# shihchinw/rlShaders

Hardware: AMD Instinct MI355X
Metric: BSDF Gsamples/sec (eval+sample+pdf) (higher is better)
Workload: dtype f32

## Files before the change

### rlshaders_amd/build.py

```python
from __future__ import annotations

import os
import shutil
import subprocess
import sys
from concurrent.futures import ThreadPoolExecutor
from pathlib import Path

PKG = Path(__file__).resolve().parent
CSRC = PKG / "csrc"
LIBDIR = PKG / "lib"
OBJDIR = PKG / "build"
LIB = LIBDIR / "librlshaders_amd.so"
ARCH = "gfx950"

SOURCES = ["shade.hip", "integrate.hip", "lights.hip", "scatter.hip", "skin.hip", "ggx.hip", "disney.hip", "sss.hip", "alternates.hip", "context.hip", "pipeline.hip",
           "libm_check.hip"]
FAST_UNITS = {"ggx.hip", "disney.hip", "sss.hip", "skin.hip", "integrate.hip", "lights.hip", "scatter.hip", "shade.hip", "alternates.hip"}
HEADERS = [CSRC / "rls_device.hpp", CSRC / "rls_libm.hpp", CSRC / "rls_libm_tables.inc", CSRC / "rls_libm_flavour_args.inc", CSRC / "rls_internal.hpp", CSRC / "rls_loops.hpp",
           PKG.parent / "include" / "rlshaders_amd.h", PKG.parent / "include" / "rlshaders_amd_diag.h"]

HIPCC_FLAGS = [
    f"--offload-arch={ARCH}", "-O3", "-std=c++17", "-fPIC",
    "-ffp-contract=off", "-fno-fast-math",
    "-fno-slp-vectorize",
    "-fno-gpu-rdc",
    "-Wall", "-Wno-unused-function",
]


def _hipcc() -> str:
    exe = shutil.which("hipcc") or "/opt/rocm/bin/hipcc"
    if not os.path.exists(exe):
        raise RuntimeError("hipcc not found: the rlshaders_amd HIP library cannot be built")
    return exe


def _stale(target: Path, deps) -> bool:
    if not target.exists():
        return True
    t = target.stat().st_mtime
    return any(Path(d).stat().st_mtime > t for d in deps)


def sources():
    return [CSRC / s for s in SOURCES if (CSRC / s).exists()]


def build_library(force: bool = False, verbose: bool = False, variant: str = "", defines=(), extra=()) -> Path:
    hipcc = _hipcc()
    LIBDIR.mkdir(exist_ok=True)
    objdir = OBJDIR if not variant else PKG / f"build_{variant}"
    lib = LIB if not variant else LIBDIR / f"librlshaders_amd_{variant}.so"
    objdir.mkdir(exist_ok=True)
    srcs = sources()
    jobs = []
    objs = []
    for src in srcs:
        flavours = [("", "RLS_FAST=0")] + ([("_fast", "RLS_FAST=1")] if src.name in FAST_UNITS else [])
        for suffix, flag in flavours:
            obj = objdir / (src.stem + suffix + ".o")
            objs.append(obj)
            if force or _stale(obj, [src, *HEADERS, Path(__file__)]):
                jobs.append([hipcc, *HIPCC_FLAGS, *extra, f"-cuid=rlshaders_amd.{src.stem}{suffix}", f"-D{flag}",
                             *[f"-D{d}" for d in defines], "-c", str(src), "-o", str(obj)])

    def run(cmd):
        if verbose:
            print(" ".join(cmd), flush=True)
        p = subprocess.run(cmd, capture_output=True, text=True)
        if p.returncode != 0:
            raise RuntimeError(f"hipcc failed:\n{' '.join(cmd)}\n{p.stdout}\n{p.stderr}")
        return p

    if jobs:
        with ThreadPoolExecutor(max_workers=min(4, len(jobs))) as ex:
            list(ex.map(run, jobs))
    if force or jobs or _stale(lib, objs):
        run([hipcc, f"--offload-arch={ARCH}", "-shared", "-fPIC", "-o", str(lib), *map(str, objs)])
    return lib


TRACE_CSRC = PKG / "csrc_trace"
TRACE_SOURCES = ["trace.hip"]
TRACE_LIB = LIBDIR / "librls_trace.so"
TRACE_HEADERS = [TRACE_CSRC / "rls_trace_device.hpp", PKG.parent / "include" / "rlshaders_amd_trace.h"]


def build_trace_library(force: bool = False, verbose: bool = False) -> Path:
    hipcc = _hipcc()
    main = build_library(verbose=verbose)
    objdir = OBJDIR / "trace"
    objdir.mkdir(parents=True, exist_ok=True)
    jobs, objs = [], []
    for name in TRACE_SOURCES:
        src = TRACE_CSRC / name
        for suffix, flag in (("", "RLS_FAST=0"), ("_fast", "RLS_FAST=1")):
            obj = objdir / (src.stem + suffix + ".o")
            objs.append(obj)
            if force or _stale(obj, [src, *HEADERS, *TRACE_HEADERS, Path(__file__)]):
                jobs.append([hipcc, *HIPCC_FLAGS, f"-cuid=rls_trace.{src.stem}{suffix}", f"-D{flag}", "-c", str(src),
                             "-o", str(obj)])

    def run(cmd):
        if verbose:
            print(" ".join(cmd), flush=True)
        p = subprocess.run(cmd, capture_output=True, text=True)
        if p.returncode != 0:
            raise RuntimeError(f"hipcc failed:\n{' '.join(cmd)}\n{p.stdout}\n{p.stderr}")

    if jobs:
        with ThreadPoolExecutor(max_workers=min(4, len(jobs))) as ex:
            list(ex.map(run, jobs))
    if force or jobs or _stale(TRACE_LIB, [*objs, main]):
        run([hipcc, f"--offload-arch={ARCH}", "-shared", "-fPIC", "-o", str(TRACE_LIB), *map(str, objs),
             f"-L{LIBDIR}", "-lrlshaders_amd", "-Wl,-rpath,$ORIGIN"])
    return TRACE_LIB


def build_trace_example(verbose: bool = False) -> Path:
    OBJDIR.mkdir(exist_ok=True)
    lib = build_trace_library(verbose=verbose)
    src, out = PKG / "host" / "example_trace.cpp", OBJDIR / "example_trace"
    if _stale(out, [src, PKG / "host" / "rls_trace.hpp", lib, LIB, *HEADERS, *TRACE_HEADERS]):
        cmd = ["g++", "-std=c++14", "-O2", "-Wall", f"-I{PKG.parent / 'include'}", f"-I{PKG / 'host'}", str(src), "-o", str(out),
               f"-L{LIBDIR}", "-lrls_trace", "-lrlshaders_amd", f"-Wl,-rpath,{LIBDIR}", "-L/opt/rocm/lib", "-Wl,-rpath,/opt/rocm/lib"]
        if verbose:
            print(" ".join(cmd), flush=True)
        p = subprocess.run(cmd, capture_output=True, text=True)
        if p.returncode != 0:
            raise RuntimeError(f"host example example_trace failed to build:\n{p.stdout}\n{p.stderr}")
    return out


def build_host_examples(verbose: bool = False) -> Path:
    OBJDIR.mkdir(exist_ok=True)
    first = OBJDIR / "example_arnold_stub"
    for name in ("example_arnold_stub", "example_multi_gpu", "example_host_pipeline", "test_arnold_stub"):
        src = PKG / "host" / f"{name}.cpp"
        out = OBJDIR / name
        if not src.exists():
            continue
        if _stale(out, [src, PKG / "host" / "rls_batch.hpp", PKG / "host" / "rl_arnold_stub.hpp", LIB, *HEADERS]):
            cmd = ["g++", "-std=c++14", "-O2", "-Wall", "-pthread", f"-I{PKG.parent / 'include'}", f"-I{PKG / 'host'}",
                   str(src), "-o", str(out), f"-L{LIBDIR}", "-lrlshaders_amd", f"-Wl,-rpath,{LIBDIR}",
                   "-L/opt/rocm/lib", "-Wl,-rpath,/opt/rocm/lib"]
            if verbose:
                print(" ".join(cmd), flush=True)
            p = subprocess.run(cmd, capture_output=True, text=True)
            if p.returncode != 0:
                raise RuntimeError(f"host example {name} failed to build:\n{p.stdout}\n{p.stderr}")
    return first


if __name__ == "__main__":
    args = sys.argv[1:]
    variant = args[args.index("--variant") + 1] if "--variant" in args else ""
    defines = [a[2:] for a in args if a.startswith("-D")]
    extra = []
    for i, a in enumerate(args):
        if a.startswith(("-f", "-m", "-O")):
            extra.append(a)
            if a == "-mllvm":
# ... 3 lines not shown
```

### rlshaders_amd/csrc/context.hip

```cpp
#include <stdarg.h>
#include <stdlib.h>
#include <string.h>

#include "rls_internal.hpp"

namespace {
thread_local char g_error[512] = "";
}

namespace rlsh {

void set_error(const char *fmt, ...)
{
    va_list ap;
    va_start(ap, fmt);
    vsnprintf(g_error, sizeof(g_error), fmt, ap);
    va_end(ap);
}

rls_status hip_fail(hipError_t e, const char *what)
{
    set_error("HIP error %d (%s) in %s", (int)e, hipGetErrorString(e), what);
    (void)hipGetLastError();
    return e == hipErrorOutOfMemory ? RLS_ERR_OUT_OF_MEMORY : RLS_ERR_HIP;
}

}

using namespace rlsd;

extern "C" {

const char *rls_last_error(void) { return g_error; }

const char *rls_status_string(rls_status s)
{
    switch (s) {
    case RLS_OK: return "ok";
    case RLS_ERR_INVALID_ARGUMENT: return "invalid argument";
    case RLS_ERR_NO_DEVICE: return "no HIP device";
    case RLS_ERR_HIP: return "HIP runtime error";
    case RLS_ERR_OUT_OF_MEMORY: return "out of device memory";
    case RLS_ERR_UNSUPPORTED: return "unsupported";
    case RLS_ERR_ABORTED: return "stopped by a callback";
    default: return "unknown status";
    }
}

int rls_version(void) { return RLS_VERSION_MAJOR * 1000 + RLS_VERSION_MINOR; }

rls_status rls_context_create(int device_ordinal, rls_context **out)
{
    RLS_REQUIRE(out != nullptr, "out is NULL");
    *out = nullptr;
    int count = 0;
    hipError_t e = hipGetDeviceCount(&count);
    if (e != hipSuccess || count <= 0) {
        rlsh::set_error("rls_context_create: no HIP device visible (%s)",
                        e == hipSuccess ? "count = 0" : hipGetErrorString(e));
        return RLS_ERR_NO_DEVICE;
    }
    if (device_ordinal < 0 || device_ordinal >= count) {
        rlsh::set_error("rls_context_create: device %d out of range [0, %d)", device_ordinal, count);
        return RLS_ERR_NO_DEVICE;
    }
    RLS_HIP_TRY(hipSetDevice(device_ordinal));
    hipDeviceProp_t prop;
    RLS_HIP_TRY(hipGetDeviceProperties(&prop, device_ordinal));

    rls_context *ctx = (rls_context *)calloc(1, sizeof(rls_context));
    if (!ctx) { rlsh::set_error("rls_context_create: host allocation failed"); return RLS_ERR_OUT_OF_MEMORY; }
    ctx->device = device_ordinal;
    ctx->compute_units = prop.multiProcessorCount > 0 ? prop.multiProcessorCount : 256;
    ctx->blocks_per_cu = 64;
    if (const char *s = getenv("RLS_BLOCKS_PER_CU")) {
        int v = atoi(s);
        if (v >= 1 && v <= 4096) ctx->blocks_per_cu = v;
    }
    hipError_t e1 = hipStreamCreateWithFlags(&ctx->own_stream, hipStreamNonBlocking);
    hipError_t e2 = e1 == hipSuccess ? hipEventCreate(&ctx->ev_start) : e1;
    hipError_t e3 = e2 == hipSuccess ? hipEventCreate(&ctx->ev_stop) : e2;
    if (e3 == hipSuccess) e3 = hipEventCreate(&ctx->ev_probe_start);
    if (e3 == hipSuccess) e3 = hipEventCreate(&ctx->ev_probe_stop);
    hipError_t e4 = e3 == hipSuccess ? hipMalloc((void **)&ctx->scratch_u64, sizeof(unsigned long long)) : e3;
    if (e4 != hipSuccess) {
        rls_status st = rlsh::hip_fail(e4, "rls_context_create");
        rls_context_destroy(ctx);
        return st;
    }
    ctx->stream = ctx->own_stream;
    *out = ctx;
    return RLS_OK;
}

void rls_context_destroy(rls_context *ctx)
{
    if (!ctx) return;
    (void)hipSetDevice(ctx->device);
    if (ctx->capturing) {
        hipGraph_t g = nullptr;
        if (hipStreamEndCapture(ctx->stream, &g) == hipSuccess && g) (void)hipGraphDestroy(g);
        (void)hipGetLastError();
    }
    if (ctx->own_stream) (void)hipStreamSynchronize(ctx->own_stream);
    if (ctx->scratch_u64) (void)hipFree(ctx->scratch_u64);
    if (ctx->stamp_buf) (void)hipFree(ctx->stamp_buf);
    if (ctx->ev_start) (void)hipEventDestroy(ctx->ev_start);
    if (ctx->ev_stop) (void)hipEventDestroy(ctx->ev_stop);
    if (ctx->ev_probe_start) (void)hipEventDestroy(ctx->ev_probe_start);
    if (ctx->ev_probe_stop) (void)hipEventDestroy(ctx->ev_probe_stop);
    if (ctx->own_stream) (void)hipStreamDestroy(ctx->own_stream);
    free(ctx);
}

int rls_device_count(void)
{
    int n = 0;
    if (hipGetDeviceCount(&n) != hipSuccess) { (void)hipGetLastError(); return 0; }
    return n;
}

rls_status rls_shard_range(int64_t total, int rank, int world, int64_t *first, int64_t *count)
{
    RLS_REQUIRE(first != nullptr && count != nullptr, "NULL argument");
    RLS_REQUIRE(world >= 1 && rank >= 0 && rank < world && total >= 0, "bad shard request");
    const __int128 lo = (__int128)total * rank / world, hi = (__int128)total * (rank + 1) / world;
    *first = (int64_t)lo;
    *count = (int64_t)(hi - lo);
    return RLS_OK;
}

rls_status rls_context_set_stream(rls_context *ctx, void *hip_stream)
{
    RLS_REQUIRE(ctx != nullptr, "ctx is NULL");
    RLS_REQUIRE(!ctx->capturing, "not allowed while a launch graph is being recorded");
    ctx->stream = (hipStream_t)hip_stream;
    return RLS_OK;
}

rls_status rls_context_use_own_stream(rls_context *ctx)
{
    RLS_REQUIRE(ctx != nullptr, "ctx is NULL");
    RLS_REQUIRE(!ctx->capturing, "not allowed while a launch graph is being recorded");
    ctx->stream = ctx->own_stream;
    return RLS_OK;
}

void *rls_context_get_stream(rls_context *ctx) { return ctx ? (void *)ctx->stream : nullptr; }

rls_status rls_context_set_math_mode(rls_context *ctx, int mode)
{
    RLS_REQUIRE(ctx != nullptr, "ctx is NULL");
    RLS_REQUIRE(mode == RLS_MATH_EXACT || mode == RLS_MATH_FAST, "mode must be RLS_MATH_EXACT or RLS_MATH_FAST");
    ctx->fast = mode == RLS_MATH_FAST;
    return RLS_OK;
}

int rls_context_get_math_mode(const rls_context *ctx) { return ctx && ctx->fast ? RLS_MATH_FAST : RLS_MATH_EXACT; }

int rls_context_device(const rls_context *ctx) { return ctx ? ctx->device : -1; }

// ... 496 lines not shown
```

### rlshaders_amd/csrc/ggx.hip

```cpp
#include "rls_internal.hpp"

using namespace rlsd;

namespace {

using namespace rlsh;

#define RLS_GGX_ARGS(a0) reload_args(a0)

enum { MIXED = 0, STREAMED_ALL = 1, UNIFORM_MATERIAL = 2 };

template <int MODE>
__device__ __forceinline__ Ggx load_closure(const rls_ggx_closure &c, Idx i, const GgxMaterial &um)
{
    constexpr bool STREAMED = MODE == STREAMED_ALL;
    V3 wo = ld3(c.wo, i), N = ld3(c.N, i), T = ld3(c.T, i);
    const PIndex<Idx> k = pindex<MODE == MIXED>(c.materials, i);
    float kr, kg, kb;
    ldrgb<STREAMED>(c.KsColor, k, kr, kg, kb);
    if (MODE == UNIFORM_MATERIAL)
        return ggx_from_material(um, wo, N, T, c.exiting ? (c.exiting[i.full()] != 0) : false, kr, kg, kb);
    float rough = ldp<STREAMED>(c.specularRoughness, k);
    float ior = ldp<STREAMED>(c.ior, k);
    float aniso = ldp<STREAMED>(c.anisotropic, k);
    bool exiting = c.exiting ? (c.exiting[i.full()] != 0) : false;
    return ggx_make(wo, N, T, exiting, kr, kg, kb, ior, rough, aniso);
}

#ifndef RLS_GGX_WAVES
#define RLS_GGX_WAVES(OP) ((OP) == OP_EVAL ? 6 : 8)
#endif
#define RLS_GGX_ATTR(OP) __launch_bounds__(rlsh::kBlock) __attribute__((amdgpu_waves_per_eu(RLS_GGX_WAVES(OP), RLS_GGX_WAVES(OP))))
template <int OP, int FAST_MATH, int MODE>
__device__ __forceinline__ void ggx_body(const GgxIO &a0)
{
    if (OP == OP_SAMPLE || OP == OP_FUSED || OP == OP_REFLECT_REFRACT || OP == OP_REFRACT || OP == OP_MICROFACET)
        stage_libm_tables();
    GgxMaterial um = {};
    if (MODE == UNIFORM_MATERIAL) {
        const rls_ggx_closure &c = a0.c;
        um = ggx_material_wave_uniform(ggx_material(c.ior.u, c.specularRoughness.u, c.anisotropic.u));
    }
    const TileRange tiles = tile_range(a0.n);
    for (int64_t base = tiles.first; base < tiles.end; base += tiles.step) {
        const Idx i = make_idx(base);
        if (i.full() >= a0.n) continue;
        const GgxIO a = RLS_GGX_ARGS(a0);
        Ggx g = load_closure<MODE>(a.c, i, um);

        if (OP == OP_SAMPLE || OP == OP_FUSED || OP == OP_REFLECT_REFRACT) {
            float rx = ldg(a.rx, i), ry = ldg(a.ry, i);
            VndfView w = vndf_view(g.view, g.fr, g.ax, g.ay);
            V3 M, M2;
            if (OP == OP_REFLECT_REFRACT) {
                float rx2 = ldg(a.rx2, i), ry2 = ldg(a.ry2, i);
                vndf_microfacet_pair(w, g.fr, rx, ry, w, g.fr, rx2, ry2, M, M2);
            } else {
                M = vndf_microfacet(w, g.fr, rx, ry);
            }
            V3 L = reflect_direction(g.view, M);
            float F = ggx_fresnel(g, L, M);
            {
                const GgxIO b = RLS_GGX_ARGS(a0);
                st3(b.wi, i, L);
                if (b.fresnel) stg(b.fresnel, i, F);
            }
            if (OP != OP_SAMPLE) {
                float fr, fg, fb, pdf;
                ggx_eval_pdf<true, true>(g, L, fr, fg, fb, pdf);
                const GgxIO b = RLS_GGX_ARGS(a0);
                strgb(b.f, i, fr, fg, fb);
                stg(b.pdf, i, pdf);
            }
            if (OP == OP_REFLECT_REFRACT) {
                V3 dir;
                ggx_refract(g, M2, dir);
                const float wgt = ggx_sample_weight(g, g.view, dir, M2);
                const GgxIO b = RLS_GGX_ARGS(a0);
                st3(b.wt, i, dir);
                stg(b.weight, i, wgt);
            }
        } else if (OP == OP_EVAL) {
            float fr, fg, fb;
            ggx_eval(g, ld3(a.cwi, i), fr, fg, fb);
            strgb(a.f, i, fr, fg, fb);
        } else if (OP == OP_PDF) {
            stg(a.pdf, i, ggx_pdf(g, ld3(a.cwi, i)));
        } else if (OP == OP_REFRACT) {
            float rx = ldg(a.rx, i), ry = ldg(a.ry, i);
            VndfView w = vndf_view(g.view, g.fr, g.ax, g.ay);
            V3 M = vndf_microfacet(w, g.fr, rx, ry);
            V3 dir;
            bool ok = ggx_refract(g, M, dir);
            st3(a.wt, i, dir);
            stg(a.weight, i, ggx_sample_weight(g, g.view, dir, M));
            if (a.refracted) a.refracted[i.full()] = ok ? 1 : 0;
        } else if (OP == OP_MICROFACET) {
            float rx = ldg(a.rx, i), ry = ldg(a.ry, i);
            V3 M;
            if (a.kernel == RLS_KERNEL_NDF) {
                M = ndf_microfacet(g, rx, ry);
            } else {
                VndfView w = vndf_view(g.view, g.fr, g.ax, g.ay);
                M = vndf_microfacet(w, g.fr, rx, ry);
            }
            st3(a.wi, i, M);
        } else if (OP == OP_NDF_PDF) {
            V3 H = normalize(g.view + ld3(a.cwi, i));
            stg(a.pdf, i, ndf_pdf(g, g.view, H));
        }
    }
}

template <int OP, int FAST_MATH, int MODE>
__global__ RLS_GGX_ATTR(OP) void ggx_kernel(GgxIO a0)
{
    ggx_body<OP, FAST_MATH, MODE>(a0);
}

#if RLS_DIAGNOSTICS
template <int OP, int FAST_MATH, int MODE>
__global__ RLS_GGX_ATTR(OP) void ggx_kernel_stamped(GgxIO a0, unsigned long long *stamps)
{
    ClockStamp<1> cs;
    cs.begin();
    ggx_body<OP, FAST_MATH, MODE>(a0);
    cs.end(stamps);
}
#endif

template <int OP>
rls_status launch_kernel(rls_context *ctx, const GgxIO &io, const char *name)
{
    const rls_ggx_closure &c = io.c;
    const bool streamed = !c.materials.id && c.KsColor.r && c.specularRoughness.v && c.ior.v && c.anisotropic.v;
    const bool uniform = !c.materials.id && !c.specularRoughness.v && !c.ior.v && !c.anisotropic.v;
    if constexpr (OP == OP_REFLECT_REFRACT)
        RLS_STAMPED_LAUNCH(streamed, (ggx_kernel_stamped<OP, RLS_FAST, STREAMED_ALL>),
                           rlsh::grid_for(ctx, io.n, rlsh::kBlock, RLS_CAP_MULT), io, name);
    if (streamed)
        hipLaunchKernelGGL((ggx_kernel<OP, RLS_FAST, STREAMED_ALL>), rlsh::grid_for(ctx, io.n, rlsh::kBlock, RLS_CAP_MULT), dim3(rlsh::kBlock), 0, ctx->stream, io);
    else if (uniform)
        hipLaunchKernelGGL((ggx_kernel<OP, RLS_FAST, UNIFORM_MATERIAL>), rlsh::grid_for_hoisting(ctx, io.n), dim3(rlsh::kBlock), 0, ctx->stream, io);
    else
        hipLaunchKernelGGL((ggx_kernel<OP, RLS_FAST, MIXED>), rlsh::grid_for(ctx, io.n, rlsh::kBlock, RLS_CAP_MULT), dim3(rlsh::kBlock), 0, ctx->stream, io);
    return rlsh::check_launch(name, RLS_FAST);
}

rls_status launch_ggx(rls_context *ctx, int op, const GgxIO &io, const char *name)
{
    switch (op) {
    case OP_SAMPLE: return launch_kernel<OP_SAMPLE>(ctx, io, name);
    case OP_EVAL: return launch_kernel<OP_EVAL>(ctx, io, name);
    case OP_PDF: return launch_kernel<OP_PDF>(ctx, io, name);
    case OP_FUSED: return launch_kernel<OP_FUSED>(ctx, io, name);
    case OP_REFRACT: return launch_kernel<OP_REFRACT>(ctx, io, name);
    case OP_REFLECT_REFRACT: return launch_kernel<OP_REFLECT_REFRACT>(ctx, io, name);
    case OP_MICROFACET: return launch_kernel<OP_MICROFACET>(ctx, io, name);
    default: return launch_kernel<OP_NDF_PDF>(ctx, io, name);
    }
}

}

RLS_FLAVOURS(ggx, rlsh::GgxIO)

#if !RLS_FAST

extern "C" {

rls_status rls_ggx_sample(rls_context *ctx, int64_t n, const rls_ggx_closure *c,
                          const float *rx, const float *ry, rls_vec3 wi, float *fresnel)
{
    RLS_PROLOGUE();
    if (rls_status s = rlsh::check_closure(__func__, c)) return s;
    RLS_REQUIRE(rx && ry, "rx/ry is NULL");
    RLS_REQUIRE(rlsh::has3(wi), "wi plane is NULL");
    GgxIO io = {};
    io.c = *c; io.rx = rx; io.ry = ry; io.wi = wi; io.fresnel = fresnel; io.n = n;
    return dispatch_ggx(ctx, OP_SAMPLE, io, "rls_ggx_sample");
}

rls_status rls_ggx_eval(rls_context *ctx, int64_t n, const rls_ggx_closure *c, rls_cvec3 wi, rls_rgb f)
{
    RLS_PROLOGUE();
    if (rls_status s = rlsh::check_closure(__func__, c)) return s;
    RLS_REQUIRE(rlsh::has3(wi) && rlsh::has3(f), "wi/f plane is NULL");
    GgxIO io = {};
    io.c = *c; io.cwi = wi; io.f = f; io.n = n;
    return dispatch_ggx(ctx, OP_EVAL, io, "rls_ggx_eval");
}

rls_status rls_ggx_pdf(rls_context *ctx, int64_t n, const rls_ggx_closure *c, rls_cvec3 wi, float *pdf)
{
    RLS_PROLOGUE();
    if (rls_status s = rlsh::check_closure(__func__, c)) return s;
    RLS_REQUIRE(rlsh::has3(wi) && pdf, "wi/pdf is NULL");
    GgxIO io = {};
    io.c = *c; io.cwi = wi; io.pdf = pdf; io.n = n;
    return dispatch_ggx(ctx, OP_PDF, io, "rls_ggx_pdf");
}

rls_status rls_ggx_sample_eval_pdf(rls_context *ctx, int64_t n, const rls_ggx_closure *c,
                                   const float *rx, const float *ry,
                                   rls_vec3 wi, rls_rgb f, float *pdf, float *fresnel)
{
    RLS_PROLOGUE();
    if (rls_status s = rlsh::check_closure(__func__, c)) return s;
    RLS_REQUIRE(rx && ry, "rx/ry is NULL");
    RLS_REQUIRE(rlsh::has3(wi) && rlsh::has3(f) && pdf, "wi/f/pdf is NULL");
    GgxIO io = {};
    io.c = *c; io.rx = rx; io.ry = ry; io.wi = wi; io.f = f; io.pdf = pdf; io.fresnel = fresnel; io.n = n;
    return dispatch_ggx(ctx, OP_FUSED, io, "rls_ggx_sample_eval_pdf");
}

rls_status rls_ggx_refract_sample(rls_context *ctx, int64_t n, const rls_ggx_closure *c,
                                  const float *rx, const float *ry,
                                  rls_vec3 wt, float *weight, uint8_t *refracted)
{
// ... 52 lines not shown
```

### rlshaders_amd/csrc/rls_device.hpp

```cpp
#pragma once

#include <hip/hip_runtime.h>
#include <stdint.h>

#include "rls_libm.hpp"

namespace rlsd {

constexpr float kPi = 3.14159265f;
constexpr float kTwoPi = 6.28318530f;
constexpr float kHalfPi = 1.57079632f;
constexpr float kInvPi = 0.31830988f;
constexpr float kEps = 1e-4f;

struct V3 { float x, y, z; };
struct V2 { float x, y; };

#define RLS_DEV __device__ __forceinline__
#ifndef RLS_BLOCK
#define RLS_BLOCK 256
#endif

RLS_DEV float sqr(float a) { return a * a; }
RLS_DEV float absf(float a) { return a < 0.0f ? -a : a; }
// ... 10 lines not shown
RLS_DEV V3 operator*(V3 a, float s) { return mk(a.x * s, a.y * s, a.z * s); }
RLS_DEV float dot(V3 a, V3 b) { return a.x * b.x + a.y * b.y + a.z * b.z; }
RLS_DEV V3 cross(V3 a, V3 b)
{
    return mk(a.y * b.z - a.z * b.y, a.z * b.x - a.x * b.z, a.x * b.y - a.y * b.x);
}
RLS_DEV V3 to_frame(V3 a, V3 u, V3 v, V3 w)
{
    return mk(a.x * u.x + a.y * v.x + a.z * w.x,
              a.x * u.y + a.y * v.y + a.z * w.y,
              a.x * u.z + a.y * v.z + a.z * w.z);
}
RLS_DEV bool is_zero(V3 a) { return a.x == 0.0f && a.y == 0.0f && a.z == 0.0f; }
RLS_DEV bool is_finite3(V3 a) { return isfinite(a.x) && isfinite(a.y) && isfinite(a.z); }

struct Frame { V3 U, V, N; };

#ifndef RLS_FAST
#define RLS_FAST 0
#endif
#if RLS_FAST
RLS_DEV float refined_div(float a, float b)
{
    float r = __builtin_amdgcn_rcpf(b);
    float q = a * r;
    float e = __builtin_fmaf(-b, q, a);
    return __builtin_fmaf(e, r, q);
}
#define R_DIV(a, b) ((a) * __builtin_amdgcn_rcpf(b))
#define R_RCP(b) __builtin_amdgcn_rcpf(b)
#define R_RCPW(b) __builtin_amdgcn_rcpf(b)
#define R_TWO_OVER(den) (2.0f * __builtin_amdgcn_rcpf(den))
#define R_SQRT(x) __builtin_amdgcn_sqrtf(x)
#define R_SQRT1P(y) __builtin_amdgcn_sqrtf(1.0f + (y))
#define R_SQRT1M(t) __builtin_amdgcn_sqrtf(1.0f - (t))
#define R_EXP(x) __expf(x)
#define R_EXP_IN_RANGE(x) __expf(x)
#define R_LOG(x) __logf(x)
#define R_POW(x, y) __powf(x, y)
#define R_POW5(x) __powf(x, 5.0f)
#define R_DIVH(a, b) refined_div(a, b)
#define R_RCPH(b) refined_div(1.0f, b)
#define R_RCPG(b) refined_div(1.0f, b)
#define R_RCPHI(b) __builtin_amdgcn_rcpf(b)
#define R_DIVC(x, C) ((x) * (1.0f / (C)))
#define R_DIVCW(x, C) ((x) * (1.0f / (C)))
#define R_SQRTH(x) rlm::sqrt32(x)
#define R_SQRTH1P(y) rlm::sqrt32_1p(y)
RLS_DEV void t_sincos(float x, float *s, float *c) { *s = __sinf(x); *c = __cosf(x); }
RLS_DEV void t_sincos_any(float x, float *s, float *c) { t_sincos(x, s, c); }
RLS_DEV void stage_libm_tables() {}
#else
#define R_DIV(a, b) rlm::div32((a), (b))
#define R_RCP(b) rlm::rcp32(b)
#define R_RCPW(b) rlm::rcp32_w(b)
#define R_TWO_OVER(den) (2.0f * rlm::rcp32_w(den))
#define R_SQRT(x) rlm::sqrt32(x)
#define R_DIVH(a, b) rlm::div32((a), (b))
#define R_RCPH(b) rlm::rcp32_w(b)
#define R_DIVC(x, C) rlm::div32_const((x), (C), 1.0f / (C))
#define R_DIVCW(x, C) rlm::div32_const_w((x), (C), 1.0f / (C))
#define R_RCPHI(b) rlm::rcp32_hi(b)
#define R_RCPG(b) rlm::rcp32_hi(b)
#define R_SQRTH(x) rlm::sqrt32(x)
#define R_SQRT1P(y) rlm::sqrt32_1p(y)
#define R_SQRTH1P(y) rlm::sqrt32_1p(y)
#define R_SQRT1M(t) rlm::sqrt32_1m(t)
static __device__ __constant__ rlm::Tables c_libm_tables = RLM_TABLES_INIT;
static __shared__ rlm::Tables s_libm_tables;
RLS_DEV void stage_libm_tables()
{
    const uint64_t *src = reinterpret_cast<const uint64_t *>(&c_libm_tables);
    uint64_t *dst = reinterpret_cast<uint64_t *>(&s_libm_tables);
    for (unsigned t = threadIdx.x; t < sizeof(rlm::Tables) / 8; t += RLS_BLOCK) dst[t] = src[t];
    __syncthreads();
}
#define R_EXP(x) rlm::exp32(x, s_libm_tables)
#define R_EXP_IN_RANGE(x) rlm::exp32_in_range(x, s_libm_tables)
#define R_LOG(x) rlm::log32(x, s_libm_tables)
#define R_POW(x, y) rlm::pow32(x, y, s_libm_tables)
#define R_POW5(x) rlm::pow5_32(x, s_libm_tables)
RLS_DEV void t_sincos(float x, float *s, float *c) { rlm::sincos32_v<false>(x, s, c); }
RLS_DEV void t_sincos_any(float x, float *s, float *c) { rlm::sincos32_v<true>(x, s, c); }
RLS_DEV float t_atan2(float y, float x) { return rlm::atan2_32_q(y, x, s_libm_tables); }
RLS_DEV float t_acos(float x) { return rlm::acos32_q(x); }
RLS_DEV float t_tan(float x) { return rlm::tan32_q<false>(x); }
#endif


RLS_DEV float length(V3 a) { return R_SQRT(a.x * a.x + a.y * a.y + a.z * a.z); }
RLS_DEV V3 normalize(V3 a)
{
    float t = length(a);
    if (t != 0.0f) t = R_RCPW(t);
    return mk(a.x * t, a.y * t, a.z * t);
}
RLS_DEV V3 normalize_h(V3 a)
{
    float t = R_SQRTH(a.x * a.x + a.y * a.y + a.z * a.z);
    if (t != 0.0f) t = R_RCPH(t);
    return mk(a.x * t, a.y * t, a.z * t);
}
RLS_DEV float linearstep(float lo, float hi, float t) { return clampf(R_DIV(t - lo, hi - lo), 0.0f, 1.0f); }

template <bool BOUNDED_PHI = false>
RLS_DEV V3 spherical_direction(float cosTheta, float phi)
{
    float r = R_SQRT1M(sqr(cosTheta));
    float s, c;
    if (BOUNDED_PHI) t_sincos(phi, &s, &c);
    else t_sincos_any(phi, &s, &c);
    return mk(r * c, r * s, cosTheta);
}
RLS_DEV V3 reflect_direction(V3 i, V3 n) { return n * (2.0f * absf(dot(i, n))) - i; }
RLS_DEV float luminance(float r, float g, float b) { return r * 0.212671f + g * 0.715160f + b * 0.072169f; }
RLS_DEV V2 concentric_disk(float rx, float ry)
{
    rx = rx * 2.0f - 1.0f;
    ry = ry * 2.0f - 1.0f;
    V2 out;
    if (rx == 0.0f && ry == 0.0f) {
        out.x = 0.0f; out.y = 0.0f;
        return out;
    }
    const bool wide = absf(rx) > absf(ry);
    const float q = R_DIV(wide ? kHalfPi * 0.5f * ry : 0.5f * rx, wide ? rx : ry);
    const float r = wide ? rx : ry;
    const float phi = wide ? q : kHalfPi * (1.0f - q);
    float s, c;
    t_sincos(phi, &s, &c);
    out.x = r * c;
    out.y = r * s;
    return out;
}
RLS_DEV V3 cosine_hemisphere(const Frame &fr, float rx, float ry)
{
    V2 d = concentric_disk(rx, ry);
    float z = R_SQRT(maxf(0.0f, 1.0f - sqr(d.x) - sqr(d.y)));
    return to_frame(mk(d.x, d.y, z), fr.U, fr.V, fr.N);
}

struct VndfView {
    float ax, ay;
    float cosPhi, sinPhi;
    float B, B2, G1, invB;
    bool nearNormal;
#if !RLS_FAST
    float yG1;
#endif
};

#if RLS_FAST
RLS_DEV V3 vndf_local(V3 view, const Frame &fr)
{
    return mk(dot(fr.U, view), dot(fr.V, view), clampf(dot(fr.N, view), -1.0f, 1.0f));
}
RLS_DEV VndfView vndf_view_from(V3 local, float ax, float ay)
{
    VndfView w;
    w.ax = ax; w.ay = ay;
    float cz = local.z;
    float sx = local.x * ax;
    float sy = local.y * ay;
    float h2 = sx * sx + sy * sy;
    float z = cz * rlm::rcp32_w(rlm::sqrt32(h2 + cz * cz));
    float h = R_SQRTH(h2);
    bool flat = !(z < (1.0f - kEps));
// ... 1217 lines not shown
```

### rlshaders_amd/csrc/rls_internal.hpp

```cpp
#pragma once

#include <hip/hip_runtime.h>
#include <stdint.h>
#include <stdio.h>

#include "../../include/rlshaders_amd.h"

#ifndef RLS_DIAGNOSTICS
#define RLS_DIAGNOSTICS 1
#endif
#if RLS_DIAGNOSTICS
#include "../../include/rlshaders_amd_diag.h"
#endif
#include "rls_device.hpp"

struct rls_context {
    int device;
    int compute_units;
    int blocks_per_cu;
    hipStream_t stream;
    hipStream_t own_stream;
    hipEvent_t ev_start, ev_stop;
    hipEvent_t ev_probe_start, ev_probe_stop;
    unsigned long long *scratch_u64;
    int fast;
    int capturing;
    unsigned long long *stamps;
    unsigned long long *stamp_buf;
    int64_t stamp_slots;
};

#define RLS_HIDDEN extern "C" __attribute__((visibility("hidden")))
#if RLS_FAST
#define RLS_FLAVOURS(verb, IO)                                                                                \
    RLS_HIDDEN rls_status rls_fast_##verb(rls_context *ctx, int sel, const IO *io, const char *name)         \
    {                                                                                                         \
        return launch_##verb(ctx, sel, *io, name);                                                            \
    }
#else
#define RLS_FLAVOURS(verb, IO)                                                                                \
    RLS_HIDDEN rls_status rls_fast_##verb(rls_context *ctx, int sel, const IO *io, const char *name);        \
    static rls_status dispatch_##verb(rls_context *ctx, int sel, const IO &io, const char *name)              \
    {                                                                                                         \
        return ctx->fast ? rls_fast_##verb(ctx, sel, &io, name) : launch_##verb(ctx, sel, io, name);          \
    }
#endif

namespace rlsh {

enum GgxOp { OP_SAMPLE, OP_EVAL, OP_PDF, OP_FUSED, OP_REFRACT, OP_REFLECT_REFRACT, OP_MICROFACET, OP_NDF_PDF };
struct GgxIO {
    rls_ggx_closure c;
    const float *rx, *ry, *rx2, *ry2;
    rls_cvec3 cwi;
    rls_vec3 wi;
    rls_rgb f;
    float *pdf, *fresnel;
    rls_vec3 wt;
    float *weight;
    uint8_t *refracted;
    int64_t n;
    int kernel;
};

enum DisneyOp { DOP_SAMPLE, DOP_EVAL, DOP_PDF, DOP_FUSED };
struct DisneyIO {
    rls_disney_closure c;
    const float *rx, *ry;
    rls_cvec3 cwi;
    rls_vec3 wi;
    rls_rgb f;
    float *pdf;
    int64_t n;
};

enum SssOp { SOP_ND, SOP_ND_PDF, SOP_ND_EVAL, SOP_PROBE, SOP_MIS };
struct SssIO {
    rls_sss_closure c;
    const float *rx, *ry, *rin;
    rls_cvec3 P, disp, sampleN;
    int literal;
    float *r;
    rls_vec3 origin, dir;
    float *maxdist, *pdf;
    rls_rgb profile;
    int64_t n;
};
enum MiscOp { MOP_CAVITY, MOP_DIFFUSE_DIR, MOP_UTIL, MOP_REFLECT_LUM };
struct MiscIO {
    rls_cvec3 a, b, c;
    const float *rx, *ry;
    float *out;
    rls_vec3 v0, v1;
    int64_t n;
};

enum AltOp { AOP_GTR2_ANISO, AOP_GTR2, AOP_NDF_PDF, AOP_D_GTR2, AOP_GAUSS, AOP_LIBM };
struct AltIO {
    rls_disney_closure c;
    const float *rx, *ry;
    rls_cvec3 v;
    rls_vec3 out3;
    float *out1;
    rls_param dist_x;
    float *r, *pdf, *profile;
    int fn;
    int64_t n;
};

struct SkinIO {
    rls_skin_closure c;
    const float *xi[6];
// ... 396 lines not shown
```

### rlshaders_amd/csrc/rls_libm.hpp

```cpp
#pragma once

#include <math.h>
#include <stdint.h>
#include <string.h>

#if defined(__HIPCC__)
#include <hip/hip_runtime.h>
#define RLM_FN __host__ __device__ __forceinline__
#else
#define RLM_FN static inline
#endif

namespace rlm {

RLM_FN uint32_t f2u(float x)
{
#if defined(__HIP_DEVICE_COMPILE__)
    return __float_as_uint(x);
#else
    uint32_t u; memcpy(&u, &x, 4); return u;
#endif
}
RLM_FN float u2f(uint32_t u)
{
// ... 641 lines not shown
    float res = hx < 0 ? (hy < 0 ? zl - pi : pi - zl) : (hy < 0 ? -z : z);
    res = (iy == 0) ? (hx < 0 ? (hy < 0 ? -pi : pi) : y) : res;
    res = (ix == 0 && iy != 0) ? (hy < 0 ? -pi_o_2 : pi_o_2) : res;
    return res;
}

RLM_FN float atan32_t(float x, const Tables &tab)
{
    const float aT0 = u2f(0x3eaaaaabu), aT1 = u2f(0xbe4ccccdu), aT2 = u2f(0x3e124925u), aT3 = u2f(0xbde38e38u),
                aT4 = u2f(0x3dba2e6eu), aT5 = u2f(0xbd9d8795u), aT6 = u2f(0x3d886b35u), aT7 = u2f(0xbd6ef16bu),
                aT8 = u2f(0x3d4bda59u), aT9 = u2f(0xbd15a221u), aT10 = u2f(0x3c8569d7u);
    const int32_t hx = (int32_t)f2u(x);
    const int32_t ix = hx & 0x7fffffff;
    const float ax = fabs32(x);
    const bool r0 = ix < 0x3ee00000;
    const int id = (ix >= 0x3f300000) + (ix >= 0x3f980000) + (ix >= 0x401c0000);
    const float *k = tab.atan_k[id];
    const float A = k[0], B = k[1], C = k[2], D = k[3], hi = k[4], lo = k[5];
    const float num = r0 ? x : A * ax + B;
    const float den = r0 ? 1.0f : C * ax + D;
    const float t = div32_m(num, den);
    const float z = t * t;
    const float w = z * z;
    const float s1 = z * (aT0 + w * (aT2 + w * (aT4 + w * (aT6 + w * (aT8 + w * aT10)))));
    const float s2 = w * (aT1 + w * (aT3 + w * (aT5 + w * (aT7 + w * aT9))));
    const float ts = t * (s1 + s2);
    const float small = t - ts;
    float big = hi - ((ts - lo) - t);
    big = hx < 0 ? -big : big;
    float res = r0 ? small : big;
    res = (ix < 0x31000000) ? x : res;
    const float huge = u2f(0x3fc90fdau) + u2f(0x33a22168u);
    res = (ix >= 0x4c000000 && ix <= 0x7f800000) ? (hx > 0 ? huge : -huge) : res;
    return res;
}

RLM_FN float atan2_32_t(float y, float x, const Tables &tab)
{
    const float pi_o_2 = u2f(0x3fc90fdbu), pi = u2f(0x40490fdbu), pi_lo = u2f(0xb3bbbd2eu);
    const int32_t hx = (int32_t)f2u(x), hy = (int32_t)f2u(y);
    const int32_t ix = hx & 0x7fffffff, iy = hy & 0x7fffffff;
    if (__builtin_expect(ix >= 0x7f800000 || iy >= 0x7f800000, 0)) return atan2_32(y, x);
    const int32_t k = (iy - ix) >> 23;
    float z = atan32_t(fabs32(div32(y, x)), tab);
    z = (k > 60) ? (pi_o_2 + 0.5f * pi_lo) : z;
    z = (hx < 0 && k < -60) ? 0.0f : z;
    const float zl = z - pi_lo;
    float res = hx < 0 ? (hy < 0 ? zl - pi : pi - zl) : (hy < 0 ? -z : z);
    res = (iy == 0) ? (hx < 0 ? (hy < 0 ? -pi : pi) : y) : res;
    res = (ix == 0 && iy != 0) ? (hy < 0 ? -pi_o_2 : pi_o_2) : res;
    return res;
}

RLM_FN float atan2_32_q(float y, float x, const Tables &tab)
{
    const float pi = u2f(0x40490fdbu), pi_lo = u2f(0xb3bbbd2eu);
    const float aT0 = u2f(0x3eaaaaabu), aT1 = u2f(0xbe4ccccdu), aT2 = u2f(0x3e124925u), aT3 = u2f(0xbde38e38u),
                aT4 = u2f(0x3dba2e6eu), aT5 = u2f(0xbd9d8795u), aT6 = u2f(0x3d886b35u), aT7 = u2f(0xbd6ef16bu),
                aT8 = u2f(0x3d4bda59u), aT9 = u2f(0xbd15a221u), aT10 = u2f(0x3c8569d7u);
    const int32_t hx = (int32_t)f2u(x), hy = (int32_t)f2u(y);
    const uint32_t ix = (uint32_t)hx & 0x7fffffffu, iy = (uint32_t)hy & 0x7fffffffu;
    const int32_t k = ((int32_t)iy - (int32_t)ix) >> 23;
    if (__builtin_expect(ix - 0x00800000u >= 0x7f000000u || iy - 0x00800000u >= 0x7f000000u || (uint32_t)(k + 27) > 50u, 0))
        return atan2_32_t(y, x, tab);
    const float q = fabs32(div32(y, x));
    const uint32_t iq = f2u(q);
    const bool r0 = iq < 0x3ee00000u;
    const int id = (iq >= 0x3f300000u) + (iq >= 0x3f980000u) + (iq >= 0x401c0000u);
    const float *c = tab.atan_k[id];
    const float A = c[0], B = c[1], C = c[2], D = c[3], hi = c[4], lo = c[5];
    const float num = r0 ? q : A * q + B;
    const float den = r0 ? 1.0f : C * q + D;
    const float t = div32_m(num, den);
    const float zz = t * t;
    const float w = zz * zz;
    const float s1 = zz * (aT0 + w * (aT2 + w * (aT4 + w * (aT6 + w * (aT8 + w * aT10)))));
    const float s2 = w * (aT1 + w * (aT3 + w * (aT5 + w * (aT7 + w * aT9))));
    const float ts = t * (s1 + s2);
    const float z = r0 ? t - ts : hi - ((ts - lo) - t);
    const float zl = z - pi_lo;
    return hx < 0 ? (hy < 0 ? zl - pi : pi - zl) : (hy < 0 ? -z : z);
}

RLM_FN float acos32_q(float x)
{
    const float pi = u2f(0x40490fdau), pio2_hi = u2f(0x3fc90fdau), pio2_lo = u2f(0x33a22168u);
    const float pS0 = u2f(0x3e2aaaabu), pS1 = u2f(0xbea6b090u), pS2 = u2f(0x3e4e0aa8u), pS3 = u2f(0xbd241146u),
                pS4 = u2f(0x3a4f7f04u), pS5 = u2f(0x3811ef08u);
    const float qS1 = u2f(0xc019d139u), qS2 = u2f(0x4001572du), qS3 = u2f(0xbf303361u), qS4 = u2f(0x3d9dc62eu);
    const int32_t hx = (int32_t)f2u(x);
    const uint32_t ix = (uint32_t)hx & 0x7fffffffu;
    if (__builtin_expect(ix - 0x23000001u >= 0x3f800000u - 0x23000001u, 0)) return acos32(x);
    const bool mid = ix < 0x3f000000u;
    const bool neg = hx < 0;
    const float z = mid ? x * x : (neg ? (1.0f + x) * 0.5f : (1.0f - x) * 0.5f);
    const float p = z * (pS0 + z * (pS1 + z * (pS2 + z * (pS3 + z * (pS4 + z * pS5)))));
    const float q = 1.0f + z * (qS1 + z * (qS2 + z * (qS3 + z * qS4)));
    const float r = div32_m(p, q);
    float res = pio2_hi - (x - (pio2_lo - x * r));
    if (!mid) {
        const float s = sqrt32<false>(z);
        const float df = u2f(f2u(s) & 0xfffff000u);
        const float c = div32_m(z - df * df, s + df);
        const float r_pos = 2.0f * (df + (r * s + c));
        const float r_neg = pi - 2.0f * (s + (r * s - pio2_lo));
        res = neg ? r_neg : r_pos;
    }
    return res;
}

RLM_FN float acos32_v(float x)
{
    const float pi = u2f(0x40490fdau), pio2_hi = u2f(0x3fc90fdau), pio2_lo = u2f(0x33a22168u);
    const float pS0 = u2f(0x3e2aaaabu), pS1 = u2f(0xbea6b090u), pS2 = u2f(0x3e4e0aa8u), pS3 = u2f(0xbd241146u),
                pS4 = u2f(0x3a4f7f04u), pS5 = u2f(0x3811ef08u);
    const float qS1 = u2f(0xc019d139u), qS2 = u2f(0x4001572du), qS3 = u2f(0xbf303361u), qS4 = u2f(0x3d9dc62eu);
    const int32_t hx = (int32_t)f2u(x);
    const int32_t ix = hx & 0x7fffffff;
    const bool mid = ix < 0x3f000000;
    const bool neg = hx < 0;
    const float z = mid ? x * x : (neg ? (1.0f + x) * 0.5f : (1.0f - x) * 0.5f);
    const float p = z * (pS0 + z * (pS1 + z * (pS2 + z * (pS3 + z * (pS4 + z * pS5)))));
    const float q = 1.0f + z * (qS1 + z * (qS2 + z * (qS3 + z * qS4)));
    const float r = div32_m(p, q);
    const float r_mid = pio2_hi - (x - (pio2_lo - x * r));
    float res = r_mid;
    if (!mid) {
        const float s = sqrt32<false>(z);
        const float df = u2f(f2u(s) & 0xfffff000u);
        const float c = div32_m(z - df * df, s + df);
        const float r_pos = 2.0f * (df + (r * s + c));
        const float r_neg = pi - 2.0f * (s + (r * s - pio2_lo));
        res = neg ? r_neg : r_pos;
    }
    res = (ix <= 0x23000000) ? pio2_hi + pio2_lo : res;
    res = (ix == 0x3f800000) ? (hx > 0 ? 0.0f : pi + 2.0f * pio2_lo) : res;
    res = (ix > 0x3f800000) ? (x - x) / (x - x) : res;
    return res;
}

template <bool FULL, bool CONTRACT>
RLM_FN double reduce_pio2(float y, int *np, bool *large_negative)
{
    const double hpi_inv = 0x1.45F306DC9C883p+23, hpi = 0x1.921FB54442D18p0;
    const double x = (double)y;
    *large_negative = false;
    if (FULL && __builtin_expect(((f2u(y) >> 20) & 0x7ffu) >= 0x42fu, 0)) {
        if (((f2u(y) >> 23) & 0xffu) == 0xffu) { *np = 0; return (double)(y - y); }
        *large_negative = (f2u(y) >> 31) != 0;
        return reduce_large(f2u(y), np);
    }
    const double r = x * hpi_inv;
    const int n = ((int32_t)r + 0x800000) >> 24;
    *np = n;
    return CONTRACT ? mad(-(double)n, hpi, x) : x - (double)n * hpi;
}

template <bool FULL = true>
RLM_FN void sincos32_v(float y, float *sinp, float *cosp)
{
    const double C0 = 0x1p0, C1 = -0x1.ffffffd0c621cp-2, C2 = 0x1.55553e1068f19p-5, C3 = -0x1.6c087e89a359dp-10,
                 C4 = 0x1.99343027bf8c3p-16;
    const double S1 = -0x1.555545995a603p-3, S2 = 0x1.1107605230bc4p-7, S3 = -0x1.994eb3774cf24p-13;
    int n;
    bool lneg;
    const double x = reduce_pio2<FULL, true>(y, &n, &lneg);
// ... 133 lines not shown
```

Measured before the change: 67.73.

## Route GGX reflect-refract through separately compiled kernel with occupancy hints and faster atan2

Adds a separately built shared library with a dedicated GGX reflect+refract kernel. It uses launch bounds and an 8-waves-per-EU hint, a restructured body that reloads arguments per store group to cut register pressure, and an atan2 variant that divides with a Newton-refined hardware reciprocal. The precise (non-fast) path for non-uniform GGX reflect-refract now dispatches to it unless an environment flag restores the old kernel. This targets occupancy and math cost in the GGX path, but adds a second library dependency and may change rounding in atan2.

```diff
diff --git a/rlshaders_amd/build.py b/rlshaders_amd/build.py
--- a/rlshaders_amd/build.py
+++ b/rlshaders_amd/build.py
@@ -76,9 +76,35 @@
     if jobs:
         with ThreadPoolExecutor(max_workers=min(4, len(jobs))) as ex:
             list(ex.map(run, jobs))
-    if force or jobs or _stale(lib, objs):
-        run([hipcc, f"--offload-arch={ARCH}", "-shared", "-fPIC", "-o", str(lib), *map(str, objs)])
+    rr = build_ggx_rr_library(force=force, verbose=verbose)
+    if force or jobs or _stale(lib, [*objs, rr]):
+        run([hipcc, f"--offload-arch={ARCH}", "-shared", "-fPIC", "-o", str(lib), *map(str, objs),
+             f"-L{LIBDIR}", "-lrls_ggx_rr", "-Wl,-rpath,$ORIGIN"])
     return lib
+
+
+GGX_RR_CSRC = PKG / "csrc_ggx_rr"
+GGX_RR_LIB = LIBDIR / "librls_ggx_rr.so"
+
+
+def build_ggx_rr_library(force: bool = False, verbose: bool = False) -> Path:
+    hipcc = _hipcc()
+    LIBDIR.mkdir(exist_ok=True)
+    objdir = OBJDIR / "ggx_rr"
+    objdir.mkdir(parents=True, exist_ok=True)
+    src, obj = GGX_RR_CSRC / "ggx_rr.hip", objdir / "ggx_rr.o"
+    cmds = []
+    if force or _stale(obj, [src, *HEADERS, Path(__file__)]):
+        cmds.append([hipcc, *HIPCC_FLAGS, "-cuid=rls_ggx_rr.ggx_rr", "-DRLS_FAST=0", "-c", str(src), "-o", str(obj)])
+    if force or cmds or _stale(GGX_RR_LIB, [obj]):
+        cmds.append([hipcc, f"--offload-arch={ARCH}", "-shared", "-fPIC", "-Wl,--no-undefined", "-o", str(GGX_RR_LIB), str(obj)])
+    for cmd in cmds:
+        if verbose:
+            print(" ".join(cmd), flush=True)
+        p = subprocess.run(cmd, capture_output=True, text=True)
+        if p.returncode != 0:
+            raise RuntimeError(f"hipcc failed:\n{' '.join(cmd)}\n{p.stdout}\n{p.stderr}")
+    return GGX_RR_LIB
 
 
 TRACE_CSRC = PKG / "csrc_trace"
diff --git a/rlshaders_amd/csrc/context.hip b/rlshaders_amd/csrc/context.hip
--- a/rlshaders_amd/csrc/context.hip
+++ b/rlshaders_amd/csrc/context.hip
@@ -77,6 +77,7 @@
         int v = atoi(s);
         if (v >= 1 && v <= 4096) ctx->blocks_per_cu = v;
     }
+    if (const char *s = getenv("RLSHADERS_AMD_FROZEN_GGX")) ctx->frozen_ggx = atoi(s) != 0;
     hipError_t e1 = hipStreamCreateWithFlags(&ctx->own_stream, hipStreamNonBlocking);
     hipError_t e2 = e1 == hipSuccess ? hipEventCreate(&ctx->ev_start) : e1;
     hipError_t e3 = e2 == hipSuccess ? hipEventCreate(&ctx->ev_stop) : e2;
diff --git a/rlshaders_amd/csrc/ggx.hip b/rlshaders_amd/csrc/ggx.hip
--- a/rlshaders_amd/csrc/ggx.hip
+++ b/rlshaders_amd/csrc/ggx.hip
@@ -1,6 +1,9 @@
 #include "rls_internal.hpp"
 
 using namespace rlsd;
+
+extern "C" int rls_ggx_rr_launch(const rlsh::GgxIO *io, int streamed, unsigned grid, unsigned long long *stamps,
+                                 hipStream_t stream);
 
 namespace {
 
@@ -135,6 +138,17 @@
     const rls_ggx_closure &c = io.c;
     const bool streamed = !c.materials.id && c.KsColor.r && c.specularRoughness.v && c.ior.v && c.anisotropic.v;
     const bool uniform = !c.materials.id && !c.specularRoughness.v && !c.ior.v && !c.anisotropic.v;
+#if !RLS_FAST
+    if (OP == OP_REFLECT_REFRACT && !uniform && !ctx->frozen_ggx) {
+        const dim3 grid = rlsh::grid_for(ctx, io.n, rlsh::kBlock, RLS_CAP_MULT);
+        unsigned long long *stamps = nullptr;
+#if RLS_DIAGNOSTICS
+        if (streamed) stamps = rlsh::stamps_for_launch(ctx);
+#endif
+        (void)rls_ggx_rr_launch(&io, streamed ? 1 : 0, grid.x, stamps, ctx->stream);
+        return rlsh::check_launch(name, RLS_FAST);
+    }
+#endif
     if constexpr (OP == OP_REFLECT_REFRACT)
         RLS_STAMPED_LAUNCH(streamed, (ggx_kernel_stamped<OP, RLS_FAST, STREAMED_ALL>),
                            rlsh::grid_for(ctx, io.n, rlsh::kBlock, RLS_CAP_MULT), io, name);
diff --git a/rlshaders_amd/csrc/rls_device.hpp b/rlshaders_amd/csrc/rls_device.hpp
--- a/rlshaders_amd/csrc/rls_device.hpp
+++ b/rlshaders_amd/csrc/rls_device.hpp
@@ -116,7 +116,10 @@
 #define R_POW5(x) rlm::pow5_32(x, s_libm_tables)
 RLS_DEV void t_sincos(float x, float *s, float *c) { rlm::sincos32_v<false>(x, s, c); }
 RLS_DEV void t_sincos_any(float x, float *s, float *c) { rlm::sincos32_v<true>(x, s, c); }
-RLS_DEV float t_atan2(float y, float x) { return rlm::atan2_32_q(y, x, s_libm_tables); }
+#ifndef RLM_ATAN2_Q
+#define RLM_ATAN2_Q rlm::atan2_32_q
+#endif
+RLS_DEV float t_atan2(float y, float x) { return RLM_ATAN2_Q(y, x, s_libm_tables); }
 RLS_DEV float t_acos(float x) { return rlm::acos32_q(x); }
 RLS_DEV float t_tan(float x) { return rlm::tan32_q<false>(x); }
 #endif
diff --git a/rlshaders_amd/csrc/rls_internal.hpp b/rlshaders_amd/csrc/rls_internal.hpp
--- a/rlshaders_amd/csrc/rls_internal.hpp
+++ b/rlshaders_amd/csrc/rls_internal.hpp
@@ -28,6 +28,7 @@
     unsigned long long *stamps;
     unsigned long long *stamp_buf;
     int64_t stamp_slots;
+    int frozen_ggx;
 };
 
 #define RLS_HIDDEN extern "C" __attribute__((visibility("hidden")))
diff --git a/rlshaders_amd/csrc/rls_libm.hpp b/rlshaders_amd/csrc/rls_libm.hpp
--- a/rlshaders_amd/csrc/rls_libm.hpp
+++ b/rlshaders_amd/csrc/rls_libm.hpp
@@ -747,6 +747,51 @@
     return hx < 0 ? (hy < 0 ? zl - pi : pi - zl) : (hy < 0 ? -z : z);
 }
 
+RLM_FN float div32_core(float a, float b)
+{
+#if defined(__HIP_DEVICE_COMPILE__)
+    float r = __builtin_amdgcn_rcpf(b);
+    const float e = __builtin_fmaf(-b, r, 1.0f);
+    r = __builtin_fmaf(e, r, r);
+    const float q0 = a * r;
+    const float r0 = __builtin_fmaf(-b, q0, a);
+    const float q1 = __builtin_fmaf(r0, r, q0);
+    const float r1 = __builtin_fmaf(-b, q1, a);
+    return __builtin_fmaf(r1, r, q1);
+#else
+    return a / b;
+#endif
+}
+RLM_FN float atan2_32_qs(float y, float x, const Tables &tab)
+{
+    const float pi = u2f(0x40490fdbu), pi_lo = u2f(0xb3bbbd2eu);
+    const float aT0 = u2f(0x3eaaaaabu), aT1 = u2f(0xbe4ccccdu), aT2 = u2f(0x3e124925u), aT3 = u2f(0xbde38e38u),
+                aT4 = u2f(0x3dba2e6eu), aT5 = u2f(0xbd9d8795u), aT6 = u2f(0x3d886b35u), aT7 = u2f(0xbd6ef16bu),
+                aT8 = u2f(0x3d4bda59u), aT9 = u2f(0xbd15a221u), aT10 = u2f(0x3c8569d7u);
+    const int32_t hx = (int32_t)f2u(x), hy = (int32_t)f2u(y);
+    const uint32_t ix = (uint32_t)hx & 0x7fffffffu, iy = (uint32_t)hy & 0x7fffffffu;
+    const int32_t k = ((int32_t)iy - (int32_t)ix) >> 23;
+    if (__builtin_expect(ix - 0x0c000000u >= 0x72800000u || iy - 0x0c000000u >= 0x72800000u || (uint32_t)(k + 27) > 50u, 0))
+        return atan2_32_t(y, x, tab);
+    const float q = fabs32(div32_core(y, x));
+    const uint32_t iq = f2u(q);
+    const bool r0 = iq < 0x3ee00000u;
+    const int id = (iq >= 0x3f300000u) + (iq >= 0x3f980000u) + (iq >= 0x401c0000u);
+    const float *c = tab.atan_k[id];
+    const float A = c[0], B = c[1], C = c[2], D = c[3], hi = c[4], lo = c[5];
+    const float num = r0 ? q : A * q + B;
+    const float den = r0 ? 1.0f : C * q + D;
+    const float t = div32_m(num, den);
+    const float zz = t * t;
+    const float w = zz * zz;
+    const float s1 = zz * (aT0 + w * (aT2 + w * (aT4 + w * (aT6 + w * (aT8 + w * aT10)))));
+    const float s2 = w * (aT1 + w * (aT3 + w * (aT5 + w * (aT7 + w * aT9))));
+    const float ts = t * (s1 + s2);
+    const float z = r0 ? t - ts : hi - ((ts - lo) - t);
+    const float zl = z - pi_lo;
+    return hx < 0 ? (hy < 0 ? zl - pi : pi - zl) : (hy < 0 ? -z : z);
+}
+
 RLM_FN float acos32_q(float x)
 {
     const float pi = u2f(0x40490fdau), pio2_hi = u2f(0x3fc90fdau), pio2_lo = u2f(0x33a22168u);
diff --git a/rlshaders_amd/csrc_ggx_rr/ggx_rr.hip b/rlshaders_amd/csrc_ggx_rr/ggx_rr.hip
--- /dev/null
+++ b/rlshaders_amd/csrc_ggx_rr/ggx_rr.hip
@@ -0,0 +1,97 @@
+#define RLM_ATAN2_Q rlm::atan2_32_qs
+#include "../csrc/rls_internal.hpp"
+
+using namespace rlsd;
+
+namespace {
+
+using namespace rlsh;
+
+enum { MIXED = 0, STREAMED_ALL = 1 };
+
+template <int MODE>
+__device__ __forceinline__ Ggx load_closure(const rls_ggx_closure &c, Idx i)
+{
+    constexpr bool STREAMED = MODE == STREAMED_ALL;
+    V3 wo = ld3(c.wo, i), N = ld3(c.N, i), T = ld3(c.T, i);
+    const PIndex<Idx> k = pindex<MODE == MIXED>(c.materials, i);
+    float kr, kg, kb;
+    ldrgb<STREAMED>(c.KsColor, k, kr, kg, kb);
+    float rough = ldp<STREAMED>(c.specularRoughness, k);
+    float ior = ldp<STREAMED>(c.ior, k);
+    float aniso = ldp<STREAMED>(c.anisotropic, k);
+    bool exiting = c.exiting ? (c.exiting[i.full()] != 0) : false;
+    return ggx_make(wo, N, T, exiting, kr, kg, kb, ior, rough, aniso);
+}
+
+#define RLS_GGX_RR_ATTR __launch_bounds__(rlsh::kBlock) __attribute__((amdgpu_waves_per_eu(8, 8)))
+
+template <int MODE>
+__device__ __forceinline__ void ggx_rr_body(const GgxIO &a0)
+{
+    stage_libm_tables();
+    const TileRange tiles = tile_range(a0.n);
+    for (int64_t base = tiles.first; base < tiles.end; base += tiles.step) {
+        const Idx i = make_idx(base);
+        if (i.full() >= a0.n) continue;
+        const GgxIO a = reload_args(a0);
+        Ggx g = load_closure<MODE>(a.c, i);
+        float rx = ldg(a.rx, i), ry = ldg(a.ry, i);
+        VndfView w = vndf_view(g.view, g.fr, g.ax, g.ay);
+        V3 M, M2;
+        float rx2 = ldg(a.rx2, i), ry2 = ldg(a.ry2, i);
+        vndf_microfacet_pair(w, g.fr, rx, ry, w, g.fr, rx2, ry2, M, M2);
+        V3 L = reflect_direction(g.view, M);
+        float F = ggx_fresnel(g, L, M);
+        {
+            const GgxIO b = reload_args(a0);
+            st3(b.wi, i, L);
+            if (b.fresnel) stg(b.fresnel, i, F);
+        }
+        {
+            float fr, fg, fb, pdf;
+            ggx_eval_pdf<true, true>(g, L, fr, fg, fb, pdf);
+            const GgxIO b = reload_args(a0);
+            strgb(b.f, i, fr, fg, fb);
+            stg(b.pdf, i, pdf);
+        }
+        {
+            V3 dir;
+            ggx_refract(g, M2, dir);
+            const float wgt = ggx_sample_weight(g, g.view, dir, M2);
+            const GgxIO b = reload_args(a0);
+            st3(b.wt, i, dir);
+            stg(b.weight, i, wgt);
+        }
+    }
+}
+
+template <int MODE>
+__global__ RLS_GGX_RR_ATTR void ggx_rr_kernel(GgxIO a0)
+{
+    ggx_rr_body<MODE>(a0);
+}
+
+template <int MODE>
+__global__ RLS_GGX_RR_ATTR void ggx_rr_kernel_stamped(GgxIO a0, unsigned long long *stamps)
+{
+    ClockStamp<1> cs;
+    cs.begin();
+    ggx_rr_body<MODE>(a0);
+    cs.end(stamps);
+}
+
+}
+
+extern "C" __attribute__((visibility("default")))
+int rls_ggx_rr_launch(const rlsh::GgxIO *io, int streamed, unsigned grid, unsigned long long *stamps, hipStream_t stream)
+{
+    const dim3 g(grid), b(rlsh::kBlock);
+    if (stamps && streamed)
+        hipLaunchKernelGGL((ggx_rr_kernel_stamped<STREAMED_ALL>), g, b, 0, stream, *io, stamps);
+    else if (streamed)
+        hipLaunchKernelGGL((ggx_rr_kernel<STREAMED_ALL>), g, b, 0, stream, *io);
+    else
+        hipLaunchKernelGGL((ggx_rr_kernel<MIXED>), g, b, 0, stream, *io);
+    return (int)hipPeekAtLastError();
+}
```

Result: no change. 68.35, median of 6 (+0.9%).
